# Lornatang/Real_ESRGAN-PyTorch

Measured on AMD Instinct MI355X. Metric: x4 SR train images/sec (256->1024), higher is better.
Workload: dtype f16; 1 GPU; RealESRNet x4 L1 train step, RRDBNet 23 blocks, LR 256^2 -> HR 1024^2, batch 16/GPU, degradation=hip, Adam+EMA, GradScaler; global_batch=16, parallelism=dp1

## Files before the change

### include/resr.h

```cpp
#ifndef RESR_H_
#define RESR_H_

#include <stddef.h>
#include <stdint.h>

#ifdef __cplusplus
extern "C" {
#endif

#define RESR_VERSION 3

typedef enum {
    RESR_OK = 0,
    RESR_ERR_ARG = -1,
    RESR_ERR_LAUNCH = -2,
    RESR_ERR_WORKSPACE = -3
} resr_status;

typedef enum { RESR_F16 = 0, RESR_F32 = 1, RESR_F16X2 = 2 } resr_dtype;

enum {
    RESR_CONV_LRELU = 1 << 0,
    RESR_CONV_UPSAMPLE_IN = 1 << 1,
    RESR_CONV_CLAMP01 = 1 << 2,
    RESR_CONV_OUT_NCHW_F32 = 1 << 3,
    RESR_CONV_MASK = 1 << 4,
    RESR_CONV_NO_BIAS = 1 << 5,
    RESR_CONV_AUX_BEFORE_MASK = 1 << 6,
    RESR_CONV_AUX_BEFORE_RES = 1 << 7,
    RESR_CONV_WRITE_SIGNBITS = 1 << 8,
    RESR_CONV_MASK_BITS = 1 << 9,
    RESR_CONV_OUT_SINGLE = 1 << 10,
    RESR_CONV_SINGLE_W16 = 1 << 11,
    RESR_CONV_MX_PAIRS = 1 << 12,
    RESR_CONV_MX_SIGNBITS = 1 << 13
};

typedef struct {
    int32_t n, h, w;
    int32_t cin;
    int32_t cin0;
    int32_t in0_stride;
    int32_t in1_stride;
    int32_t cout;
    int32_t cout_pad;
    int32_t out_stride;
    int32_t res0_stride, res1_stride, mask_stride;
    int32_t dtype;
    int32_t flags;
    float s0, t0, s1, t1, slope;
    int32_t in0_chunk_stride, in1_chunk_stride, out_chunk_stride;
    int32_t res0_chunk_stride, res1_chunk_stride, mask_chunk_stride;
    int64_t in0_lo_offset, in1_lo_offset, out_lo_offset, res0_lo_offset, res1_lo_offset;
    int32_t s2d_in_channels, s2d_out_channels, cout_groups;
    int32_t x2_pair_chunks;
    int32_t reserved2_;
    int64_t mask_lo_offset;
    int64_t in0_q_offset, in1_q_offset, out_q_offset, w_mx_offset;
} ResrConvDesc;

int resr_conv3x3(const ResrConvDesc* d, const void* in0, const void* in1, const void* w_packed,
                 const float* bias, const void* res0, const void* res1, const void* mask,
                 void* out, void* aux_out, void* stream);

size_t resr_conv3x3_chain_state_bytes(int32_t n, int32_t h, int32_t w);
int resr_conv3x3_chain(int32_t njobs, const ResrConvDesc* descs, const void* in0, const void* in1,
                       const void* const* packed_w, const float* const* bias, const void* const* mask,
                       void* const* out, void* const* aux_out, void* chain_state, size_t chain_state_bytes, void* stream);
// ... 210 lines not shown
```

### real_esrgan-pytorch_amd/_lib.py

```python
from __future__ import annotations

import ctypes as C
import os

_HERE = os.path.dirname(os.path.abspath(__file__))
LIB_PATH = os.environ.get("RESR_LIB_PATH") or os.path.join(_HERE, "csrc", "libresr_hip.so")

RESR_F16, RESR_F32, RESR_F16X2 = 0, 1, 2
CONV_LRELU, CONV_UPSAMPLE_IN, CONV_CLAMP01, CONV_OUT_NCHW_F32, CONV_MASK, CONV_NO_BIAS = 1, 2, 4, 8, 16, 32
CONV_AUX_BEFORE_MASK, CONV_AUX_BEFORE_RES = 64, 128
CONV_WRITE_SIGNBITS = 1 << 8
CONV_MASK_BITS = 1 << 9
CONV_OUT_SINGLE = 1 << 10
CONV_SINGLE_W16 = 1 << 11
X2_PLAN_GROWTH_F16_INFER, X2_PLAN_GROWTH_GRAD_F16, X2_PLAN_GROWTH_GRAD_STORE_F16, X2_PLAN_GROWTH_ACT_F16_WGRAD = 1, 2, 4, 8
X2_PLAN_GROWTH_ACT_G_HI_WGRAD = 16
X2_PLAN_GROWTH_W16_INFER = 32
X2_PLAN_MX_INFER = 64
X2_PLAN_MX_BWD = 128
X2_PLAN_F16_BACKWARD = 256
X2_PLAN_MX_WGRAD = 512
X2_PLAN_MX_TAIL = 1024
X2_PLAN_MX_TRAIN_FORWARD = 2048
X2_PLAN_OUTPUT_PARITY = (X2_PLAN_GROWTH_F16_INFER | X2_PLAN_GROWTH_W16_INFER | X2_PLAN_MX_INFER | X2_PLAN_F16_BACKWARD
# ... 6 lines not shown
    (512, 128 + 8, "MX_WGRAD (512) rides on MX_BWD (128: the gradient planes' q tensors) + GROWTH_ACT_F16_WGRAD (8: the stream chunks are the pair chunks)"),
    (1024, 512 + 128 + 8, "MX_TAIL (1024) extends MX_WGRAD (512) to the 4x-resolution tail"),
    (2048, 1 + 32 + 64 + 256, "MX_TRAIN_FORWARD (2048) runs the inference MX forward (1 + 32 + 64) in training, in front of the f16 backward pass (256)"),
)


def x2_plan_error(plan: int):
    if not 0 <= plan <= 4095:
        return ("x2_plan must be a bit set of X2_PLAN_GROWTH_F16_INFER (1) | X2_PLAN_GROWTH_GRAD_F16 (2) | X2_PLAN_GROWTH_GRAD_STORE_F16 (4) | "
                "X2_PLAN_GROWTH_ACT_F16_WGRAD (8) | X2_PLAN_GROWTH_ACT_G_HI_WGRAD (16) | X2_PLAN_GROWTH_W16_INFER (32) | X2_PLAN_MX_INFER (64) | "
                f"X2_PLAN_MX_BWD (128) | X2_PLAN_F16_BACKWARD (256) | X2_PLAN_MX_WGRAD (512) | X2_PLAN_MX_TAIL (1024) | X2_PLAN_MX_TRAIN_FORWARD (2048), got {plan}")
    if (plan & X2_PLAN_MX_BWD) and (plan & X2_PLAN_GROWTH_GRAD_STORE_F16):
        return f"x2_plan={plan}: MX_BWD (128) reads the growth-plane gradients as pairs; GROWTH_GRAD_STORE_F16 (4) stores them single"
    for bit, needs, text in X2_PLAN_RULES:
        if (plan & bit) and (plan & needs) != needs:
            return f"x2_plan={plan}: {text}"
    return None


def x2_plan_f16_backward(plan: int) -> bool:
    return bool(plan & X2_PLAN_F16_BACKWARD)


def x2_plan_packs_mx(plan: int, training: bool) -> bool:
    return bool(plan & ((X2_PLAN_MX_BWD | X2_PLAN_MX_TRAIN_FORWARD) if training else X2_PLAN_MX_INFER))


def x2_plan_layout_key(plan: int) -> int:
    return plan & (X2_PLAN_MX_INFER | X2_PLAN_MX_BWD | X2_PLAN_MX_WGRAD | X2_PLAN_MX_TAIL | X2_PLAN_MX_TRAIN_FORWARD)


CONV_MX_PAIRS = 1 << 12
CONV_MX_SIGNBITS = 1 << 13
RESR_VERSION = 3


class ConvDesc(C.Structure):
    _fields_ = [("n", C.c_int32), ("h", C.c_int32), ("w", C.c_int32),
                ("cin", C.c_int32), ("cin0", C.c_int32), ("in0_stride", C.c_int32), ("in1_stride", C.c_int32),
                ("cout", C.c_int32), ("cout_pad", C.c_int32), ("out_stride", C.c_int32),
                ("res0_stride", C.c_int32), ("res1_stride", C.c_int32), ("mask_stride", C.c_int32),
                ("dtype", C.c_int32), ("flags", C.c_int32),
                ("s0", C.c_float), ("t0", C.c_float), ("s1", C.c_float), ("t1", C.c_float), ("slope", C.c_float),
                ("in0_chunk_stride", C.c_int32), ("in1_chunk_stride", C.c_int32), ("out_chunk_stride", C.c_int32),
                ("res0_chunk_stride", C.c_int32), ("res1_chunk_stride", C.c_int32), ("mask_chunk_stride", C.c_int32),
                ("in0_lo_offset", C.c_int64), ("in1_lo_offset", C.c_int64), ("out_lo_offset", C.c_int64),
                ("res0_lo_offset", C.c_int64), ("res1_lo_offset", C.c_int64),
                ("s2d_in_channels", C.c_int32), ("s2d_out_channels", C.c_int32), ("cout_groups", C.c_int32),
                ("x2_pair_chunks", C.c_int32), ("reserved2_", C.c_int32), ("mask_lo_offset", C.c_int64),
                ("in0_q_offset", C.c_int64), ("in1_q_offset", C.c_int64), ("out_q_offset", C.c_int64), ("w_mx_offset", C.c_int64)]


class WgradDesc(C.Structure):
    _fields_ = [("n", C.c_int32), ("h", C.c_int32), ("w", C.c_int32),
                ("cin", C.c_int32), ("cin0", C.c_int32), ("in0_stride", C.c_int32), ("in1_stride", C.c_int32),
                ("cin_real", C.c_int32), ("cout", C.c_int32), ("cout_pad", C.c_int32), ("g_stride", C.c_int32),
                ("dtype", C.c_int32), ("flags", C.c_int32), ("splits", C.c_int32), ("scale", C.c_float),
                ("x_lo_offset", C.c_int64), ("g_lo_offset", C.c_int64), ("x_chunk_stride", C.c_int64), ("g_chunk_stride", C.c_int64)]


class PackChunk(C.Structure):
    _fields_ = [("src_off", C.c_int64), ("dst_off", C.c_int64), ("src_cout", C.c_int32), ("src_cin", C.c_int32),
                ("m_off", C.c_int32), ("m_count", C.c_int32), ("k_off", C.c_int32), ("k_count", C.c_int32),
                ("mt", C.c_int32), ("transposed", C.c_int32), ("scale", C.c_float), ("virtual4x4", C.c_int32),
                ("scale_ptr", C.c_void_p)]

# ... 173 lines not shown
```

### real_esrgan-pytorch_amd/csrc/conv3x3.h

```cpp
#pragma once
#include "common.h"

namespace resr {

struct ConvArgs {
    const char* in0;
    const char* in1;
    const char* w;
    const float* bias;
    const char* res0;
    const char* res1;
    const char* mask;
    char* out;
    uint8_t* aux;
    int n, h, w_, hs, ws;
    int cin, cin0;
    int in0_stride_b, in1_stride_b;
    int cout;
    int out_stride, res0_stride, res1_stride, mask_stride;
    size_t in0_chunk_b, in1_chunk_b;
    int out_chunk, res0_chunk, res1_chunk, mask_chunk;
    int flags;
    float s0, t0, s1, t1, slope;
    int tiles_x, tiles_y;
// ... 19 lines not shown
    const float* bias;
    char* out;
    void* aux;
    int cin;
    int dep;
    int kind;
    int w_mt, w_m;
    int pad_;
    const char* res0;
    const char* res1;
    float s0, t0, s1, t1;
    long out_lo, res0_lo, res1_lo;
    const char* w_mx;
    long out_q;
};
constexpr int kMaxChain = 6;
constexpr int kMaxBiasGroups = 8;
constexpr int kChainHdr = 16;
struct ChainArgs {
    int njobs;
    unsigned cap;
    unsigned* state;
    unsigned* host_errors;
    const char* nan16;
    int split[kMaxChain + 2];
    ChainJob job[kMaxChain];
};
struct ChainNone {};

inline double conv_algorithmic_bytes(const ConvArgs& a, size_t es) {
    const double px_out = (double)a.n * a.h * a.w_, px_in = (double)a.n * a.hs * a.ws;
    const int pair_ch = (es == 4 && a.pair_chunks > 0 && a.pair_chunks * 32 < a.cin) ? a.pair_chunks * 32 : a.cin;
    double b = px_in * (pair_ch * (double)es + (a.cin - pair_ch) * 2.0);
    const bool nchw = a.flags & RESR_CONV_OUT_NCHW_F32;
    b += px_out * a.cout * (nchw ? 4 : (es == 4 && a.out_single) ? 2 : es);
    if (a.flags & RESR_CONV_MASK) b += px_out * ((a.flags & RESR_CONV_MASK_BITS) ? ((a.cout + 31) / 32) * 4.0 : a.cout * (double)es);
    if (a.res0) b += px_out * a.cout * es;
    if (a.res1) b += px_out * a.cout * es;
    if (a.out_q) b += px_out * a.cout * 2.0;
    if (a.aux) b += px_out * ((a.flags & RESR_CONV_WRITE_SIGNBITS) ? ((a.cout + 31) / 32) * 4.0 : nchw ? a.cout : a.cout * (double)es);
    return b;
}

template <int SPP>
__device__ __forceinline__ int swz(int hx) {
    if constexpr (SPP == 4) return (hx >> 2) & 3;
    else return (hx >> 1) & 7;
}

template <typename T>
struct Frag;
template <>
struct Frag<half_t> {
    static __device__ __forceinline__ float16v mma(const uint4& a, const uint4& b, float16v c) {
        return __builtin_amdgcn_mfma_f32_32x32x16_f16(__builtin_bit_cast(half8, a),
                                                      __builtin_bit_cast(half8, b), c, 0, 0, 0);
    }
    static __device__ __forceinline__ float ld(const char* p, int idx) {
        return (float)reinterpret_cast<const half_t*>(p)[idx];
    }
};
template <>
struct Frag<float> {
    static __device__ __forceinline__ float16v mma(const uint4& a, const uint4& b, float16v c) {
        const float4v fa = __builtin_bit_cast(float4v, a), fb = __builtin_bit_cast(float4v, b);
        c = __builtin_amdgcn_mfma_f32_32x32x2f32(fa[0], fb[0], c, 0, 0, 0);
// ... 37 lines not shown
```

### real_esrgan-pytorch_amd/csrc/conv3x3.hip

```cpp
#include <stdlib.h>

#include <type_traits>

#include "conv3x3.h"

namespace resr {

template <typename T, int MT, int NT, int NW>
__global__ __launch_bounds__(64 * NW) void conv3x3_kernel(const ConvArgs a) {
    constexpr int NTHR = 64 * NW;
    constexpr int E = 16 / (int)sizeof(T);
    constexpr int SPP = 32 / E;
    constexpr int KS = SPP / 2;
    constexpr int PB = 32 * (int)sizeof(T);
    constexpr int TH = NW * NT, TW = 32, HH = TH + 2, HW = TW + 2;
    constexpr int NSLOT = HH * HW * SPP;
    constexpr int NS = (NSLOT + NTHR - 1) / NTHR;
    constexpr int BUF = HH * HW * PB;
    constexpr int WTAP = KS * MT * 1024;

    extern __shared__ __attribute__((aligned(16))) char smem[];

    const int tid = threadIdx.x, lane = tid & 63, wave = tid >> 6;
    const int bid = xcd_remap(blockIdx.x, gridDim.x);
// ... 234 lines not shown

int conv3x3_ws_f16(const ConvArgs& a, int mt, bool x2, hipStream_t stream);
bool conv3x3_ws_supported(const ConvArgs& a);
bool conv3x3_chain_device_ok();

int conv3x3_ws_chain_f16(const ConvArgs& a, const ChainJob* jobs, int njobs, const double* flop, const double* bytes, bool x2, void* state, size_t state_bytes,
                         hipStream_t stream);
static int conv3x3_route(const ResrConvDesc* d, ConvArgs& a, bool have_bias, bool have_in1, hipStream_t stream);

static int conv3x3_args(const ResrConvDesc* d, const void* in0, const void* in1, const void* w,
                        const float* bias, const void* res0, const void* res1, const void* mask,
                        void* out, void* aux, ConvArgs& a) {
    if (!d || !in0 || !w || !out) return fail(RESR_ERR_ARG, "conv3x3: null argument");
    if (d->cin <= 0 || (d->cin & 31) || (d->cin0 & 31) || d->cin0 <= 0 || d->cin0 > d->cin)
        return fail(RESR_ERR_ARG, "conv3x3: cin=%d cin0=%d must be positive multiples of 32", d->cin, d->cin0);
    if (d->cin0 < d->cin && !in1) return fail(RESR_ERR_ARG, "conv3x3: in1 missing for cin0 < cin");
    if (d->cout_pad != 32 && d->cout_pad != 64) return fail(RESR_ERR_ARG, "conv3x3: cout_pad=%d", d->cout_pad);
    if (d->cout <= 0 || d->cout > d->cout_pad) return fail(RESR_ERR_ARG, "conv3x3: cout=%d", d->cout);
    if (!(d->flags & RESR_CONV_OUT_NCHW_F32) && (d->cout & 3))
        return fail(RESR_ERR_ARG, "conv3x3: NHWC output needs cout %% 4 == 0");
    if (d->n <= 0 || d->h <= 0 || d->w <= 0) return fail(RESR_ERR_ARG, "conv3x3: empty shape");
    if ((d->flags & RESR_CONV_UPSAMPLE_IN) && ((d->h | d->w) & 1))
        return fail(RESR_ERR_ARG, "conv3x3: upsampled input needs even h,w");
    if ((d->flags & RESR_CONV_MASK) && !mask) return fail(RESR_ERR_ARG, "conv3x3: mask missing");
    if (d->flags & RESR_CONV_WRITE_SIGNBITS) {
        if (!aux || (d->cout & 7) || res0 || res1 ||
            (d->flags & (RESR_CONV_MASK | RESR_CONV_OUT_NCHW_F32 | RESR_CONV_CLAMP01 | RESR_CONV_AUX_BEFORE_MASK | RESR_CONV_AUX_BEFORE_RES)))
            return fail(RESR_ERR_ARG, "conv3x3: WRITE_SIGNBITS needs aux_out, cout %% 8 == 0 and a plain (bias/LeakyReLU) epilogue");
    }
    if (d->flags & RESR_CONV_MASK_BITS) {
        if (!(d->flags & RESR_CONV_MASK) || (d->cout & 7) || res0 || res1 || aux ||
            (d->flags & (RESR_CONV_OUT_NCHW_F32 | RESR_CONV_CLAMP01 | RESR_CONV_WRITE_SIGNBITS)))
            return fail(RESR_ERR_ARG, "conv3x3: MASK_BITS goes with MASK, cout %% 8 == 0, no residuals / aux");
    }
    const size_t es = elem_size(d->dtype);
    memset(&a, 0, sizeof(a));
    a.in0 = (const char*)in0; a.in1 = (const char*)in1; a.w = (const char*)w; a.bias = bias;
    a.res0 = (const char*)res0; a.res1 = (const char*)res1; a.mask = (const char*)mask;
    a.out = (char*)out; a.aux = (uint8_t*)aux;
    a.n = d->n; a.h = d->h; a.w_ = d->w;
    const bool up = d->flags & RESR_CONV_UPSAMPLE_IN;
    a.hs = up ? d->h / 2 : d->h; a.ws = up ? d->w / 2 : d->w;
    a.cin = d->cin; a.cin0 = d->cin0;
    a.in0_stride_b = (int)(d->in0_stride * es); a.in1_stride_b = (int)(d->in1_stride * es);
    a.cout = d->cout; a.out_stride = d->out_stride;
    a.res0_stride = d->res0_stride; a.res1_stride = d->res1_stride; a.mask_stride = d->mask_stride;
    auto chunk = [](int32_t v) { return v > 0 ? v : 32; };
    a.in0_chunk_b = (size_t)chunk(d->in0_chunk_stride) * es; a.in1_chunk_b = (size_t)chunk(d->in1_chunk_stride) * es;
    a.out_chunk = chunk(d->out_chunk_stride); a.res0_chunk = chunk(d->res0_chunk_stride);
    a.res1_chunk = chunk(d->res1_chunk_stride); a.mask_chunk = chunk(d->mask_chunk_stride);
    a.flags = d->flags & ~(RESR_CONV_OUT_SINGLE | RESR_CONV_SINGLE_W16 | RESR_CONV_MX_PAIRS | RESR_CONV_MX_SIGNBITS); a.s0 = d->s0; a.t0 = d->t0; a.s1 = d->s1; a.t1 = d->t1; a.slope = d->slope;
    a.s2d_c = 0; a.tap_c = 0; a.ngroups = 1; a.w_group_b = 0;
    a.pair_chunks = d->cin / 32; a.out_single = 0;
    a.mask_lo = (d->dtype == RESR_F16X2 && mask && (d->flags & RESR_CONV_MASK) && !(d->flags & RESR_CONV_MASK_BITS)) ? (long)d->mask_lo_offset : 0L;
    if (a.mask_lo < 0) return fail(RESR_ERR_ARG, "conv3x3: mask_lo_offset=%ld", a.mask_lo);
    if (d->dtype == RESR_F16X2) {
        if (d->x2_pair_chunks < 0 || d->x2_pair_chunks > d->cin / 32)
            return fail(RESR_ERR_ARG, "conv3x3: x2_pair_chunks=%d of %d chunks", d->x2_pair_chunks, d->cin / 32);
        if (d->x2_pair_chunks > 0) a.pair_chunks = d->x2_pair_chunks;
        if ((d->flags & RESR_CONV_SINGLE_W16) && a.pair_chunks * 32 < d->cin) a.single_stages = 1;
        if (d->flags & RESR_CONV_OUT_SINGLE) {
            if (d->flags & RESR_CONV_OUT_NCHW_F32) return fail(RESR_ERR_ARG, "conv3x3: OUT_SINGLE is an NHWC f16 output");
            a.out_single = 1;
        }
        if (d->in0_q_offset < 0 || d->in1_q_offset < 0 || d->out_q_offset < 0 || d->w_mx_offset < 0)
            return fail(RESR_ERR_ARG, "conv3x3: negative q / MX offset");
// ... 56 lines not shown
                     void* out, void* aux, hipStream_t stream) {
    ConvArgs a;
    const int rc = conv3x3_args(d, in0, in1, w, bias, res0, res1, mask, out, aux, a);
    if (rc) return rc;
    return conv3x3_route(d, a, bias != nullptr, in1 != nullptr, stream);
}

static int conv3x3_route(const ResrConvDesc* d, ConvArgs& a, bool have_bias, bool have_in1, hipStream_t stream) {
    const size_t es = elem_size(d->dtype);
    const void* in1 = have_in1 ? (const void*)a.in1 : nullptr;
    const void* res0 = a.res0;
    const void* res1 = a.res1;
    const int groups = d->cout_groups > 1 ? d->cout_groups : 1;
    (void)have_bias;
    const int mt = d->cout_pad / 32;
    if (d->dtype == RESR_F16X2) {
        const bool nchw = d->flags & RESR_CONV_OUT_NCHW_F32;
        const bool in1_pairs = in1 && d->cin0 < d->cin && a.pair_chunks * 32 > d->cin0;
        if (d->in0_lo_offset == 0 || (in1_pairs && d->in1_lo_offset == 0) || (!nchw && !a.out_single && d->out_lo_offset == 0) ||
            (res0 && d->res0_lo_offset == 0) || (res1 && d->res1_lo_offset == 0))
            return fail(RESR_ERR_ARG, "conv3x3: RESR_F16X2 needs the hi -> lo offset of every pair operand");
        a.in0_lo_b = (size_t)d->in0_lo_offset * es; a.in1_lo_b = (size_t)d->in1_lo_offset * es;
        a.out_lo = a.out_single ? 0L : (long)d->out_lo_offset; a.res0_lo = (long)d->res0_lo_offset; a.res1_lo = (long)d->res1_lo_offset;
        if (!conv3x3_ws_supported(a))
            return fail(RESR_ERR_ARG, "conv3x3: RESR_F16X2 needs tensors below 4 GB / 2^24 pixels and cout %% 8 == 0");
        if (a.mx && (a.s2d_c > 0 || a.tap_c > 0)) return fail(RESR_ERR_ARG, "conv3x3: RESR_CONV_MX_PAIRS with sparse taps");
        return conv3x3_ws_f16(a, mt, true, stream);
    }
    const long tiles4 = (long)((d->w + 31) / 32) * ((d->h + 15) / 16) * d->n;
    const bool big = tiles4 >= 512;
    if (d->dtype == RESR_F16) {
        static const char* old_env = getenv("RESR_CONV_ONE_ROLE");
        if (!old_env && conv3x3_ws_supported(a)) return conv3x3_ws_f16(a, mt, false, stream);
        if (groups > 1) return fail(RESR_ERR_ARG, "conv3x3: cout_groups > 1 needs the producer/consumer kernel's preconditions");
        if (mt == 1) return big ? launch_conv<half_t, 1, 2, 8>(a, stream) : launch_conv<half_t, 1, 2, 4>(a, stream);
        return launch_conv<half_t, 2, 2, 4>(a, stream);
    } else if (d->dtype == RESR_F32) {
        if (mt == 1) return launch_conv<float, 1, 2>(a, stream);
        return launch_conv<float, 2, 2>(a, stream);
    }
    return fail(RESR_ERR_ARG, "conv3x3: dtype=%d", d->dtype);
}

int conv3x3_block_dispatch(int njobs, const ResrConvDesc* d, const void* in0, const void* in1, const void* const* w,
                           const float* const* bias, const void* const* mask, void* const* out, void* const* aux,
                           const ResrConvDesc* d5, const void* w5, const float* bias5, const void* res0_5, const void* res1_5,
                           void* out5, void* chain_state, size_t chain_state_bytes, hipStream_t stream) {
    if (njobs <= 0 || njobs > 4 || !d) return fail(RESR_ERR_ARG, "conv3x3_chain: njobs=%d", njobs);
    ConvArgs a[4], a5;
    for (int j = 0; j < njobs; ++j) {
        const int rc = conv3x3_args(&d[j], in0, in1, w[j], bias ? bias[j] : nullptr, nullptr, nullptr, mask ? mask[j] : nullptr,
                                    out[j], aux ? aux[j] : nullptr, a[j]);
        if (rc) return rc;
    }
    if (d5) {
        const int rc = conv3x3_args(d5, in0, in1, w5, bias5, res0_5, res1_5, nullptr, out5, nullptr, a5);
        if (rc) return rc;
    }
    const char* no_chain = getenv("RESR_CONV_NO_CHAIN");
    const bool x2 = d[0].dtype == RESR_F16X2;
    bool ok = !no_chain && chain_state && njobs >= 2 && (d[0].dtype == RESR_F16 || x2) && conv3x3_chain_device_ok();
    if (ok && x2) {
        const size_t es2 = 2;
        for (int j = 0; j < njobs; ++j) {
            const bool in1_pairs = in1 && d[j].cin0 < d[j].cin && a[j].pair_chunks * 32 > d[j].cin0;
            if (d[j].dtype != RESR_F16X2 || d[j].in0_lo_offset == 0 || (d[j].out_lo_offset == 0 && !a[j].out_single) || (in1_pairs && d[j].in1_lo_offset == 0)) { ok = false; break; }
// ... 119 lines not shown
```

### real_esrgan-pytorch_amd/csrc/conv3x3_ws.h

```cpp
#pragma once
#include <stdlib.h>

#include <type_traits>

#include "conv3x3.h"

#ifndef RESR_TIMING_TAPS
#define RESR_TIMING_TAPS 9
#endif
#if defined(RESR_TRACE) && RESR_TRACE == 2
#define RESR_TRACE_STAMPS 192
#else
#define RESR_TRACE_STAMPS 64
#endif
#ifndef RESR_TIMING_VALU
#define RESR_TIMING_VALU 0
#endif

namespace resr {

static __device__ uint4 g_conv_zero16 = {0, 0, 0, 0};

extern unsigned long long* g_conv_trace;

// ... 165 lines not shown
            else a.trace[((blockIdx.x >> 4) * 2 + role) * RESR_TRACE_STAMPS + tk++] = __builtin_amdgcn_s_memrealtime();
        }
    };
    auto stamp_dump = [&](int role) {
        if constexpr (CH != 0) {
            if (a.trace && (blockIdx.x & 15) == 0 && blockIdx.x < 512 && lane == 0 && wave <= NWC)
                for (int i = 0; i < tk; ++i)
                    a.trace[((blockIdx.x >> 4) * 2 + role) * RESR_TRACE_STAMPS + i] = reinterpret_cast<const unsigned long long*>(smem + C::CHAIN_OFF + C::CHAIN_TRACE)[role * RESR_TRACE_STAMPS + i];
        }
    };

    if (wave == 0 || wave == NWC) stamp(wave == 0 ? 1 : 0);

    float* bias_lds = reinterpret_cast<float*>(smem + C::NHB * BUF);
    if (wave == 0) {
        const bool f_bias = !(a.flags & RESR_CONV_NO_BIAS) && a.bias != nullptr;
        bias_lds[lane] = (f_bias && lane < a.cout) ? a.bias[lane] * (X2 ? kLoScale : 1.f) : 0.f;
    }
    if constexpr (MT == 2 && CH == 0) {
        if (a.ngroups > 1 && !(a.flags & RESR_CONV_NO_BIAS) && a.bias != nullptr) {
            float* gb = reinterpret_cast<float*>(smem + C::GB_OFF);
            for (int i = tid; i < a.ngroups * 64 && i < kMaxBiasGroups * 64; i += C::NTHR)
                gb[i] = a.bias[i] * (X2 ? kLoScale : 1.f);
        }
    }
    if constexpr (CH) {
        float* cb = reinterpret_cast<float*>(smem + C::CHAIN_OFF);
        if (wave < kMaxChain && lane < 32) {
            const float* bp = wave < cj.njobs ? cj.job[wave].bias : nullptr;
            cb[wave * 32 + lane] = (bp && !(a.flags & RESR_CONV_NO_BIAS) && lane < a.cout) ? bp[lane] * (X2 ? kLoScale : 1.f) : 0.f;
        }
        if (wave == 0 && lane == 0) *reinterpret_cast<unsigned*>(smem + C::CHAIN_OFF + kMaxChain * 128) = 0u;
    }
    constexpr bool FAST = EPI == 0 || EPI == 2 || EPI == 6 || EPI == 16 || EPI == 33 || EPI == 128;
    if constexpr (EPI == 128) {
        if (wave == 1) reinterpret_cast<float*>(smem + C::LUT_OFF)[lane] = lane < a.cout ? a.prelu[lane] : 0.f;
    }
    if constexpr (FAST && EPI == 33) {
        if (wave == 1 && lane < 16) {
            float4v m;
#pragma unroll
            for (int r = 0; r < 4; ++r) m[r] = (((lane >> r) & 1) ? 1.f : a.slope) * (X2 ? kLoInv : 1.f);
            *reinterpret_cast<float4v*>(smem + C::LUT_OFF + lane * 16) = m;
        }
    }
    if (wave >= NWC) {
        const int pw = wave - NWC;
        if constexpr (C::NHB == 3) {
            const int ups3 = (a.flags & RESR_CONV_UPSAMPLE_IN) ? 1 : 0;
            constexpr int REM = NI - (NIP - 1) * NP;
            static_assert(NIP < 64, "vmcnt is 6 bits");
            unsigned cst[NIP], pix[NIP];
            unsigned long long val[NIP], inb[NIP];
            const unsigned lds_base = (unsigned)(size_t)(__attribute__((address_space(3))) char*)smem;
            auto dma_s = [&](const char* sbase, unsigned voff, unsigned dst, unsigned long long mask) {
                unsigned long long save;
                asm volatile("s_mov_b64 %0, exec\n\ts_mov_b64 exec, %1\n\ts_mov_b32 m0, %2\n\ts_nop 0\n\t"
                             "global_load_lds_dwordx4 %3, %4\n\ts_mov_b64 exec, %0"
                             : "=&s"(save) : "s"(mask), "s"(dst), "v"(voff), "s"(sbase) : "memory", "m0");
            };
            auto dma_v = [&](const char* src, unsigned dst, unsigned long long mask) {
                unsigned long long save;
                asm volatile("s_mov_b64 %0, exec\n\ts_mov_b64 exec, %1\n\ts_mov_b32 m0, %2\n\ts_nop 0\n\t"
                             "global_load_lds_dwordx4 %3, off\n\ts_mov_b64 exec, %0"
                             : "=&s"(save) : "s"(mask), "s"(dst), "v"(src) : "memory", "m0");
            };
#pragma unroll
// ... 692 lines not shown
            const int x = x0 + lx_e;
            const unsigned xc = (unsigned)(x < e.w_ ? x : e.w_ - 1);
            const bool f_lrelu = own && (e.flags & RESR_CONV_LRELU);
            const float2v sl2 = {e.slope, e.slope};
            const unsigned kh16 = (unsigned)kh_e * 16u;
            constexpr bool RESc = R0c || R1c;
            constexpr int NB = (RESc && MT == 2 && !(X2 && R1c)) ? 2 : 1;
            uint4v rr0[NB][MT][2], rr1[NB][MT][2];
            uint4v rr0l[X2 ? NB : 1][MT][2], rr1l[X2 ? NB : 1][MT][2];
            auto row_pix = [&](int t) {
                const int y = y0 + row0 + t;
                return ((unsigned)n * e.h + (unsigned)(y < e.h ? y : e.h - 1)) * e.w_ + xc;
            };
            auto piece_ok = [&](int m, int j) { return m * 32 + (2 * j + kh_e) * 8 < e.cout; };
            auto request = [&](int b, int t) {
                const unsigned p = row_pix(t);
#pragma unroll
                for (int m = 0; m < MT; ++m)
#pragma unroll
                    for (int j = 0; j < 2; ++j) {
                        const bool pair_ok = m * 32 + j * 16 < e.cout;
                        if (r0) {
                            const char* q0 = e.res0 + ((size_t)p * e.res0_stride + goff + (pair_ok ? (size_t)m * e.res0_chunk + j * 16 : (size_t)0)) * 2 + kh16;
                            rr0[b][m][j] = *reinterpret_cast<const uint4v*>(q0);
                            if constexpr (X2) rr0l[b][m][j] = *reinterpret_cast<const uint4v*>(q0 + e.res0_lo * 2);
                        }
                        if (r1) {
                            const char* q1 = e.res1 + ((size_t)p * e.res1_stride + goff + (pair_ok ? (size_t)m * e.res1_chunk + j * 16 : (size_t)0)) * 2 + kh16;
                            rr1[b][m][j] = *reinterpret_cast<const uint4v*>(q1);
                            if constexpr (X2) rr1l[b][m][j] = *reinterpret_cast<const uint4v*>(q1 + e.res1_lo * 2);
                        }
                    }
            };
            asm volatile("s_nop 7\n\ts_nop 7\n\ts_nop 3");
            if (r0 || r1) request(0, 0);
#pragma unroll
            for (int t = 0; t < NT; ++t) {
                const int y = y0 + row0 + t;
                const bool in_img = y < e.h && x < e.w_;
                const unsigned p = row_pix(t);
                const int b = NB == 2 ? (t & 1) : 0;
                if constexpr (NB == 2) {
                    if (t + 1 < NT) request((t + 1) & 1, t + 1);
                } else {
                    if ((r0 || r1) && t > 0) request(0, t);
                }
                char* const orow = e.out + ((size_t)p * e.out_stride + goff) * 2 + kh16;
#pragma unroll
                for (int m = 0; m < MT; ++m) {
                    unsigned sacc[2] = {0u, 0u};
                    unsigned wk = 0;
                    if constexpr (EMB) {
                        if (own) wk = mword[t][m] >> (kh_e * 8);
                    }
#pragma unroll
                    for (int j = 0; j < 2; ++j) {
                        float16v& A = acc[m][t];
                        float v0 = A[8 * j + 0], v1 = A[8 * j + 1], v2 = A[8 * j + 2], v3 = A[8 * j + 3];
                        float v4 = A[8 * j + 4], v5 = A[8 * j + 5], v6 = A[8 * j + 6], v7 = A[8 * j + 7];
                        permlane32_swap4(v0, v1, v2, v3, v4, v5, v6, v7);
                        float2v q[4] = {{v0, v1}, {v2, v3}, {v4, v5}, {v6, v7}};
                        if (EMB && own) {
                            const char* lut = smem + C::LUT_OFF;
                            const float4v ma = *reinterpret_cast<const float4v*>(lut + ((wk >> (16 * j)) & 15u) * 16);
                            const float4v mb = *reinterpret_cast<const float4v*>(lut + ((wk >> (16 * j + 4)) & 15u) * 16);
                            q[0] *= float2v{ma[0], ma[1]};
// ... 457 lines not shown
```

### real_esrgan-pytorch_amd/csrc/conv3x3_ws.hip

```cpp
#include <stdlib.h>

#include <mutex>

#include "conv3x3.h"

namespace resr {

unsigned long long* g_conv_trace = nullptr;
void conv_trace_set(void* p) { g_conv_trace = (unsigned long long*)p; }

int conv3x3_ws_mt1(const ConvArgs& a, int tile_rows, hipStream_t stream);
int conv3x3_ws_mt2(const ConvArgs& a, int tile_rows, hipStream_t stream);
int conv3x3_ws_x2_mt1(const ConvArgs& a, int tile_rows, hipStream_t stream);
int conv3x3_ws_x2_mt2(const ConvArgs& a, int tile_rows, hipStream_t stream);
int conv3x3_ws_mx_mt1(const ConvArgs& a, int tile_rows, hipStream_t stream);
int conv3x3_ws_mx_mt2(const ConvArgs& a, int tile_rows, hipStream_t stream);

bool conv3x3_chain_device_ok() {
    static int ok_dev[kMaxDevices] = {0};
    int dev = 0;
    if (hipGetDevice(&dev) != hipSuccess || dev < 0 || dev >= kMaxDevices) return false;
    if (!ok_dev[dev]) {
        hipDeviceProp_t prop;
        ok_dev[dev] = (hipGetDeviceProperties(&prop, dev) == hipSuccess && prop.multiProcessorCount == 256) ? 1 : -1;
// ... 92 lines not shown
            if (hipEventCreateWithFlags(&c.ev, hipEventDisableTiming) != hipSuccess ||
                hipHostMalloc(&hp, 64, hipHostMallocMapped) != hipSuccess || hipHostGetDevicePointer(&dp, hp, 0) != hipSuccess ||
                hipGetSymbolAddress(&np, HIP_SYMBOL(g_conv_nan16)) != hipSuccess || !np)
                return fail(RESR_ERR_LAUNCH, "conv3x3_chain: per-device set-up failed");
            memset(hp, 0, 64);
            c.err_host = (unsigned*)hp; c.err_dev = (unsigned*)dp; c.nan16 = (const char*)np;
            c.init = true;
        }
        hipStreamCaptureStatus cap = hipStreamCaptureStatusNone;
        if (hipStreamIsCapturing(stream, &cap) != hipSuccess) cap = hipStreamCaptureStatusNone;
        const bool capturing = cap == hipStreamCaptureStatusActive;
        if (!capturing) {
            if (c.owned && c.owner != stream && hipStreamWaitEvent(stream, c.ev, 0) != hipSuccess)
                return fail(RESR_ERR_LAUNCH, "conv3x3_chain: hipStreamWaitEvent");
            c.owner = stream;
            c.owned = true;
        }
        cj.state = (unsigned*)state;
        cj.cap = (unsigned)(state_bytes / sizeof(unsigned) - kChainHdr);
        cj.host_errors = c.err_dev;
        cj.nan16 = c.nan16;
        cj.njobs = njobs;
        memcpy(cj.split, split, sizeof(split));
        double f = 0, b = 0;
        for (int j = 0; j < njobs; ++j) { cj.job[j] = jobs[j]; f += flop[j]; b += bytes[j]; }
        for (int j = njobs; j < kMaxChain; ++j) cj.job[j] = jobs[njobs - 1];
        const int kind = (a.flags & RESR_CONV_MASK_BITS) ? 2 : (a.flags & RESR_CONV_WRITE_SIGNBITS) ? 1 : 0;
        const int rc = conv3x3_ws_chain_launch(a, cj, rows, kind, x2, f, b, stream);
        if (rc == RESR_OK && !capturing && hipEventRecord(c.ev, stream) != hipSuccess) return fail(RESR_ERR_LAUNCH, "conv3x3_chain: hipEventRecord");
        return rc;
    }
}

int conv3x3_ws_f16(const ConvArgs& a, int mt, bool x2, hipStream_t stream) {
    static const int rows1[] = {16, 8}, rows2[] = {16, 8};
    if (mt == 2 && (a.s2d_c > 0 || a.tap_c > 0) && !a.res0 && !a.res1 && !a.mask && !a.aux &&
        !(a.flags & ~(RESR_CONV_LRELU | RESR_CONV_NO_BIAS)) && a.cin0 == a.cin && (!(a.flags & RESR_CONV_LRELU) || (a.slope >= 0.f && a.slope <= 1.f)))
        return conv3x3_ws_sparse(a, 8, a.s2d_c > 0 ? 1 : 2, x2, stream);
    if (x2 && a.mx) {
        if (mt == 1) return conv3x3_ws_mx_mt1(a, pick_rows(a, rows1, 2), stream);
        return conv3x3_ws_mx_mt2(a, pick_rows(a, rows2, 2), stream);
    }
    if (x2) {
        if (mt == 1) return conv3x3_ws_x2_mt1(a, pick_rows(a, rows1, 2), stream);
        return conv3x3_ws_x2_mt2(a, pick_rows(a, rows2, 2), stream);
    }
    if (mt == 1) return conv3x3_ws_mt1(a, pick_rows(a, rows1, 2), stream);
    return conv3x3_ws_mt2(a, pick_rows(a, rows2, 2), stream);
}

}
```

### real_esrgan-pytorch_amd/csrc/generator.hip

```cpp
#include <stdlib.h>
#include <vector>

#include "common.h"
#include "wgrad.h"

namespace resr {

int conv3x3_dispatch(const ResrConvDesc*, const void*, const void*, const void*, const float*, const void*,
                     const void*, const void*, void*, void*, hipStream_t);
size_t wgrad_batch_partial_bytes(const WgradConv*, int, int, int);
int conv3x3_block_dispatch(int njobs, const ResrConvDesc* d, const void* in0, const void* in1, const void* const* w,
                           const float* const* bias, const void* const* mask, void* const* out, void* const* aux,
                           const ResrConvDesc* d5, const void* w5, const float* bias5, const void* res0_5, const void* res1_5,
                           void* out5, void* chain_state, size_t chain_state_bytes, hipStream_t stream);
size_t conv3x3_chain_state_bytes(int, int, int);
int wgrad_batch(const WgradConv*, int, int, int, int, int, int, int, float*, hipStream_t);
int wgrad_batch_jobs(const WgradConv*, int, int);
int wgrad_batch_quads(const WgradConv*, int, int);
int wgrad_tile_rows(int dtype);
int wgrad_x2_products();
int absmax_dispatch(const float*, long, unsigned*, int, hipStream_t);
int nchw_to_nhwc_q_dispatch(const float*, void*, int, int, int, int, int, int, int, const uint8_t*, hipStream_t, long, const unsigned*, long);
int nhwc_to_nchw_scaled_dispatch(const void*, float*, int, int, int, int, int, int, int, hipStream_t, long, const unsigned*);
int sumpool2x2_dispatch(const void*, void*, const void*, int, int, int, int, int, float, hipStream_t, long, long);
// ... 547 lines not shown
}

int generator_backward(const ResrGeneratorDesc* d, const float* gy, const float* params, const void* packed,
                       void* workspace, size_t workspace_bytes, float* grad, float* gx, hipStream_t st,
                       void* const* events, int n_events) {
    (void)params;
    Plan p;
    if (!build_plan(d, p)) return RESR_ERR_ARG;
    if (n_events != 0 && (!events || n_events != d->n_blocks + 2))
        return fail(RESR_ERR_ARG, "generator_backward: grad_ready_events needs n_blocks + 2 = %d events, got %d", d->n_blocks + 2, n_events);
    auto ready = [&](int i) -> int {
        if (n_events == 0) return RESR_OK;
        if (!events[i]) return fail(RESR_ERR_ARG, "generator_backward: null event %d", i);
        if (hipEventRecord((hipEvent_t)events[i], st) != hipSuccess) return fail(RESR_ERR_LAUNCH, "generator_backward: hipEventRecord");
        return RESR_OK;
    };
    if (!d->training) return fail(RESR_ERR_ARG, "generator_backward: forward was not run with training=1");
    if (!gy || !packed || !workspace || !grad) return fail(RESR_ERR_ARG, "generator_backward: null argument");
    Bufs b;
    carve(p, (char*)workspace, b);
    if (b.total > workspace_bytes) return fail(RESR_ERR_WORKSPACE, "generator_backward: workspace %zu < %zu", workspace_bytes, b.total);
    const X2Plan& xp = p.x2;
    const int dt = xp.f16_backward ? (int)RESR_F16 : d->dtype;
    Plan pb = p;
    pb.d.dtype = dt;
    const size_t es = elem_size(dt);
    const bool x2 = dt == RESR_F16X2;
    const size_t wes = es * (x2 ? 3 : 1);
    const int wm = x2 ? wgrad_x2_products() : 1;
    const char* no_prescale = getenv("RESR_X2_NO_GRAD_PRESCALE");
    const char* pre_t = getenv("RESR_X2_GRAD_PRESCALE_LOG2");
    const int pre_log2 = pre_t ? atoi(pre_t) : 6;
    const unsigned* gsc = (dt != RESR_F32 && !no_prescale) ? b.gscale : nullptr;
    const char* pk = (const char*)packed;
    const int N = d->n, h = p.h, w = p.w;
    const int H4 = 4 * h, W4 = 4 * w, H2 = 2 * h, W2 = 2 * w;
    if ((long)N * h * w * 32 * 16 > 0x7fffffffL) return fail(RESR_ERR_ARG, "generator: batch x resolution too large for 32-bit chunk strides");
    const int plane = N * h * w * 32;
    const int pl2 = 4 * plane, pl4 = 16 * plane;
    auto LO = [&](long planes, long pl) -> long { return x2 ? planes * pl : 0; };
    const long lo_ws = LO(6, plane), lo_t = LO(2, plane), lo_gs = LO(4, plane), lo_2 = LO(2, pl2), lo_4 = LO(2, pl4), lo_g4 = LO(1, pl4);
    const long lo_xin = x2 ? (long)N * h * w * p.ci_pad : 0;

    auto wconv = [&](const ConvSpec& c, const void* x0, int cin, int s0, const void* g, int gstride, float scale,
                     long x_lo, long g_lo) {
        WgradConv wc;
        wc.x0 = x0; wc.cin = cin; wc.in0_stride = s0; wc.cin_real = c.cin;
        wc.g = g; wc.cout = c.cout; wc.cout_pad = c.cout_pad; wc.g_stride = gstride;
        wc.x_chunk_stride = wc.g_chunk_stride = 0;
        wc.x_lo_off = x_lo; wc.g_lo_off = g_lo; wc.x_s2d_c = 0; wc.g_lo_bias_only = 0;
        wc.dw = grad + c.w_off; wc.db = grad + c.b_off; wc.scale = scale;
        wc.unscale = gsc;
        return wc;
    };
    auto wgrad_run = [&](const WgradConv* wc, int nconv, int hh, int ww, int flags) -> int {
        const int njobs = wgrad_batch_jobs(wc, nconv, dt);
        const int splits = splits_for(pb, njobs, hh, ww, x2 ? wgrad_batch_quads(wc, nconv, dt) : 0);
        if (wgrad_batch_partial_bytes(wc, nconv, splits, dt) > b.partial_bytes)
            return fail(RESR_ERR_WORKSPACE, "wgrad slab buffer too small");
        return wgrad_batch(wc, nconv, N, hh, ww, dt, flags, splits, b.partial, st);
    };
    auto wgrad = [&](const ConvSpec& c, int hh, int ww, const void* x0, int cin, int s0, const void* g, int gstride,
                     int flags, float scale, long x_chunk, long g_chunk, long x_lo, long g_lo, long x_q = 0, long g_q = 0) -> int {
        WgradConv wc = wconv(c, x0, cin, s0, g, gstride, scale, x_lo, g_lo);
        wc.x_chunk_stride = x_chunk; wc.g_chunk_stride = g_chunk;
        wc.x_q_off = x_q; wc.g_q_off = g_q;
// ... 5 lines not shown
        cd.in0_lo_offset = lo0; cd.in1_lo_offset = lo1; cd.out_lo_offset = lo_out;
        return cd;
    };

    if (gsc) RUN(absmax_dispatch(gy, (long)N * d->out_channels * H4 * W4, b.gscale, pre_log2, st));
    RUN(nchw_to_nhwc_q_dispatch(gy, b.g4, N, d->out_channels, H4, W4, 1, 32, dt, b.ymask, st, lo_g4, gsc, xp.mx_tail ? 2 * lo_g4 : 0L));
    const char* pk_mx = xp.mx_bwd ? pk + generator_mx_offset(d) : nullptr;
    auto MXT = [&](ResrConvDesc& cd, size_t pk_off, long in_q, long out_q) {
        if (!xp.mx_tail) return;
        cd.flags |= RESR_CONV_MX_PAIRS;
        cd.in0_q_offset = in_q; cd.out_q_offset = out_q;
        cd.w_mx_offset = (int64_t)((pk_mx + pk_off * 2) - (pk + pk_off * wes));
    };
    {
        const ConvSpec& c = p.convs[p.i_conv4];
        RUN(wgrad(c, H4, W4, b.c3, 64, 32, b.g4, 32, 0, 1.f, pl4, 0, lo_4, lo_g4, xp.mx_tail ? 2 * lo_4 : 0, xp.mx_tail ? 2 * lo_g4 : 0));
        ResrConvDesc cd = dgrad(H4, W4, 32, 32, 32, 0, 64, 64, 32, RESR_CONV_MASK | RESR_CONV_MASK_BITS, lo_g4, 0, lo_4);
        cd.out_chunk_stride = pl4;
        MXT(cd, p.pk_bwd_conv4, 2 * lo_g4, 2 * lo_4);
        RUN(conv3x3_dispatch(&cd, b.g4, nullptr, pk + p.pk_bwd_conv4 * wes, nullptr, nullptr, nullptr, b.bits_c3, b.gA, nullptr, st));
    }
    {
        const ConvSpec& c = p.convs[p.i_conv3];
        RUN(wgrad(c, H4, W4, b.u2, 64, 32, b.gA, 32, 0, 1.f, pl4, pl4, lo_4, lo_4, xp.mx_tail ? 2 * lo_4 : 0, xp.mx_tail ? 2 * lo_4 : 0));
        ResrConvDesc cd = dgrad(H4, W4, 64, 32, 64, 0, 64, 64, 32, RESR_CONV_MASK | RESR_CONV_MASK_BITS, lo_4, 0, lo_4);
        cd.in0_chunk_stride = pl4; cd.out_chunk_stride = pl4;
        MXT(cd, p.pk_bwd_conv3, 2 * lo_4, 2 * lo_4);
        RUN(conv3x3_dispatch(&cd, b.gA, nullptr, pk + p.pk_bwd_conv3 * wes, nullptr, nullptr, nullptr, b.bits_u2, b.gB, nullptr, st));
    }
    if (debug_stop() == 1) return RESR_OK;
    {
        const ConvSpec& c = p.convs[p.i_up2];
        RUN(wgrad(c, H4, W4, b.u1, 64, 32, b.gB, 32, RESR_CONV_UPSAMPLE_IN, 1.f, pl2, pl4, lo_2, lo_4, xp.mx_tail ? 2 * lo_2 : 0, xp.mx_tail ? 2 * lo_4 : 0));
        ResrConvDesc cd = dgrad(H4, W4, 64, 32, 64, 0, 64, 64, 32, 0, lo_4, 0, lo_4);
        cd.in0_chunk_stride = pl4; cd.out_chunk_stride = pl4;
        MXT(cd, p.pk_bwd_up2, 2 * lo_4, 0);
        RUN(conv3x3_dispatch(&cd, b.gB, nullptr, pk + p.pk_bwd_up2 * wes, nullptr, nullptr, nullptr, nullptr, b.gA, nullptr, st));
        for (int q = 0; q < 2; ++q)
            RUN(sumpool2x2_dispatch(b.gA + (size_t)q * pl4 * es, b.gM1 + (size_t)q * pl2 * es, b.u1 + (size_t)q * pl2 * es,
                                    N, H2, W2, 32, dt, 0.2f, st, lo_4, lo_2));
    }
    if (debug_stop() == 2) return RESR_OK;
    {
        const ConvSpec& c = p.convs[p.i_up1];
        RUN(wgrad(c, H2, W2, b.feat, 64, 32, b.gM1, 32, RESR_CONV_UPSAMPLE_IN, 1.f, plane, pl2, lo_t, lo_2));
        ResrConvDesc cd = dgrad(H2, W2, 64, 32, 64, 0, 64, 64, 32, 0, lo_2, 0, lo_2);
        cd.in0_chunk_stride = pl2; cd.out_chunk_stride = pl2;
        RUN(conv3x3_dispatch(&cd, b.gM1, nullptr, pk + p.pk_bwd_up1 * wes, nullptr, nullptr, nullptr, nullptr, b.gA, nullptr, st));
        for (int q = 0; q < 2; ++q)
            RUN(sumpool2x2_dispatch(b.gA + (size_t)q * pl2 * es, b.gF + (size_t)q * plane * es, nullptr, N, h, w, 32, dt, 0.2f, st,
                                    lo_2, lo_t));
    }
    if (debug_stop() == 3) return RESR_OK;
    int cur = 0;
    {
        const ConvSpec& c = p.convs[p.i_conv2];
        RUN(wgrad(c, h, w, b.trunk_out, 64, 32, b.gF, 32, 0, 1.f, plane, plane, lo_t, lo_t));
        ResrConvDesc cd = dgrad(h, w, 64, 32, 64, 0, 64, 64, 32, 0, lo_t, 0, lo_t);
        cd.in0_chunk_stride = plane; cd.out_chunk_stride = plane;
        if (xp.mx_bwd) cd.out_q_offset = 2 * lo_t;
        RUN(conv3x3_dispatch(&cd, b.gF, nullptr, pk + p.pk_bwd_conv2 * wes, nullptr, nullptr, nullptr, nullptr, b.gT[0], nullptr, st));
    }
    auto MXB = [&](ResrConvDesc& cd, size_t pk_off, long out_q) {
        if (!xp.mx_bwd) return;
        cd.flags |= RESR_CONV_MX_PAIRS;
        cd.x2_pair_chunks = 0;
        cd.in0_q_offset = 2 * lo_t; cd.in1_q_offset = 2 * lo_gs; cd.out_q_offset = out_q;
        cd.w_mx_offset = (int64_t)((pk_mx + pk_off * 2) - (pk + pk_off * wes));
    };
    RUN(ready(0));
    int e_idx = 0;
    const bool batch_rrdb = 78 * wm <= kWgradMaxJobs && !getenv("RESR_WGRAD_PER_BLOCK");
    WgradConv wc[15];
    for (int r = p.nrdb - 1; r >= 0; --r) {
        const int pos = r % 3;
        if (pos == 2) e_idx = cur;
        const char* gin = b.gT[cur];
        const char* act = b.ws[r];
        char* gS = b.gS[pos];
        const float fold = pos == 2 ? 0.04f : 0.2f;
        WgradConv* wcb = wc + (batch_rrdb ? 5 * pos : 0);
// ... 65 lines not shown
```

Before: 131.4 images/sec.

## Fuse 2x2 sum-pool and LeakyReLU mask into upsample dgrad epilogue

Adds a POOL2X2_OUT epilogue to the warp-specialized f16 conv kernel. It sums each 2x2 output cell in registers using DPP lane swaps, optionally applies the pooled LeakyReLU mask, and writes the quarter-resolution gradient directly. The two upsample-conv backward passes now use it when the dtype is f16, which removes the full-resolution gradient write and the separate sumpool kernels' read-back. The cost is extra epilogue register pressure and a narrower set of supported configurations.

Result: no change. 132.1 images/sec, median of 6 (+0.6%).

```diff
diff --git a/include/resr.h b/include/resr.h
--- a/include/resr.h
+++ b/include/resr.h
@@ -33,7 +33,8 @@
     RESR_CONV_OUT_SINGLE = 1 << 10,
     RESR_CONV_SINGLE_W16 = 1 << 11,
     RESR_CONV_MX_PAIRS = 1 << 12,
-    RESR_CONV_MX_SIGNBITS = 1 << 13
+    RESR_CONV_MX_SIGNBITS = 1 << 13,
+    RESR_CONV_POOL2X2_OUT = 1 << 14
 };
 
 typedef struct {
diff --git a/real_esrgan-pytorch_amd/_lib.py b/real_esrgan-pytorch_amd/_lib.py
--- a/real_esrgan-pytorch_amd/_lib.py
+++ b/real_esrgan-pytorch_amd/_lib.py
@@ -62,6 +62,7 @@
 
 CONV_MX_PAIRS = 1 << 12
 CONV_MX_SIGNBITS = 1 << 13
+CONV_POOL2X2_OUT = 1 << 14
 RESR_VERSION = 3
 
 
diff --git a/real_esrgan-pytorch_amd/csrc/conv3x3.h b/real_esrgan-pytorch_amd/csrc/conv3x3.h
--- a/real_esrgan-pytorch_amd/csrc/conv3x3.h
+++ b/real_esrgan-pytorch_amd/csrc/conv3x3.h
@@ -75,6 +75,8 @@
     const double px_out = (double)a.n * a.h * a.w_, px_in = (double)a.n * a.hs * a.ws;
     const int pair_ch = (es == 4 && a.pair_chunks > 0 && a.pair_chunks * 32 < a.cin) ? a.pair_chunks * 32 : a.cin;
     double b = px_in * (pair_ch * (double)es + (a.cin - pair_ch) * 2.0);
+    if (a.flags & RESR_CONV_POOL2X2_OUT)
+        return b + px_out / 4 * a.cout * (double)es * ((a.flags & RESR_CONV_MASK) ? 2 : 1);
     const bool nchw = a.flags & RESR_CONV_OUT_NCHW_F32;
     b += px_out * a.cout * (nchw ? 4 : (es == 4 && a.out_single) ? 2 : es);
     if (a.flags & RESR_CONV_MASK) b += px_out * ((a.flags & RESR_CONV_MASK_BITS) ? ((a.cout + 31) / 32) * 4.0 : a.cout * (double)es);
diff --git a/real_esrgan-pytorch_amd/csrc/conv3x3.hip b/real_esrgan-pytorch_amd/csrc/conv3x3.hip
--- a/real_esrgan-pytorch_amd/csrc/conv3x3.hip
+++ b/real_esrgan-pytorch_amd/csrc/conv3x3.hip
@@ -290,6 +290,12 @@
         if (!(d->flags & RESR_CONV_MASK) || (d->cout & 7) || res0 || res1 || aux ||
             (d->flags & (RESR_CONV_OUT_NCHW_F32 | RESR_CONV_CLAMP01 | RESR_CONV_WRITE_SIGNBITS)))
             return fail(RESR_ERR_ARG, "conv3x3: MASK_BITS goes with MASK, cout %% 8 == 0, no residuals / aux");
+    }
+    if (d->flags & RESR_CONV_POOL2X2_OUT) {
+        if (d->dtype != RESR_F16 || d->cout != 64 || d->cout_pad != 64 || ((d->h | d->w) & 1) || res0 || res1 || aux || d->out_q_offset != 0 ||
+            d->cout_groups > 1 || d->s2d_in_channels > 0 || d->s2d_out_channels > 0 ||
+            (d->flags & ~(RESR_CONV_POOL2X2_OUT | RESR_CONV_NO_BIAS | RESR_CONV_MASK)))
+            return fail(RESR_ERR_ARG, "conv3x3: POOL2X2_OUT needs f16, cout = cout_pad = 64, even h and w, a plain epilogue (bias, pooled f16 mask) and no out_q / groups / sparse taps");
     }
     const size_t es = elem_size(d->dtype);
     memset(&a, 0, sizeof(a));
@@ -412,6 +418,7 @@
     if (d->dtype == RESR_F16) {
         static const char* old_env = getenv("RESR_CONV_ONE_ROLE");
         if (!old_env && conv3x3_ws_supported(a)) return conv3x3_ws_f16(a, mt, false, stream);
+        if (d->flags & RESR_CONV_POOL2X2_OUT) return fail(RESR_ERR_ARG, "conv3x3: POOL2X2_OUT needs the producer/consumer kernel's preconditions");
         if (groups > 1) return fail(RESR_ERR_ARG, "conv3x3: cout_groups > 1 needs the producer/consumer kernel's preconditions");
         if (mt == 1) return big ? launch_conv<half_t, 1, 2, 8>(a, stream) : launch_conv<half_t, 1, 2, 4>(a, stream);
         return launch_conv<half_t, 2, 2, 4>(a, stream);
diff --git a/real_esrgan-pytorch_amd/csrc/conv3x3_ws.h b/real_esrgan-pytorch_amd/csrc/conv3x3_ws.h
--- a/real_esrgan-pytorch_amd/csrc/conv3x3_ws.h
+++ b/real_esrgan-pytorch_amd/csrc/conv3x3_ws.h
@@ -221,7 +221,8 @@
         }
         if (wave == 0 && lane == 0) *reinterpret_cast<unsigned*>(smem + C::CHAIN_OFF + kMaxChain * 128) = 0u;
     }
-    constexpr bool FAST = EPI == 0 || EPI == 2 || EPI == 6 || EPI == 16 || EPI == 33 || EPI == 128;
+    constexpr bool FAST = EPI == 0 || EPI == 2 || EPI == 6 || EPI == 16 || EPI == 33 || EPI == 128 || EPI == 256 || EPI == 257;
+    static_assert(!(EPI & 256) || (EPI <= 257 && sizeof(T) == 2 && MT == 2 && (NT & 1) == 0 && !X2 && !SP && !CH), "pooled epilogue: f16, cout 64, even rows per wave");
     if constexpr (EPI == 128) {
         if (wave == 1) reinterpret_cast<float*>(smem + C::LUT_OFF)[lane] = lane < a.cout ? a.prelu[lane] : 0.f;
     }
@@ -980,6 +981,88 @@
                         }
                     }
             };
+            if constexpr ((EPI & 256) != 0) {
+                constexpr bool PM = (EPI & 1) != 0;
+                constexpr int NC = NT / 2;
+                const int ho = e.h >> 1, wo = e.w_ >> 1;
+                const unsigned xo = xc >> 1;
+                auto cell_pix = [&](int c) {
+                    const int yo = (y0 + row0 + 2 * c) >> 1;
+                    return ((unsigned)n * ho + (unsigned)(yo < ho ? yo : ho - 1)) * wo + xo;
+                };
+                uint4v mk[PM ? NC : 1][MT][2];
+                if constexpr (PM) {
+                    const char* const mbase = ep->mask;
+                    const int m_stride = ep->mask_stride, m_chunk = ep->mask_chunk;
+#pragma unroll
+                    for (int c = 0; c < NC; ++c) {
+                        const unsigned p2 = cell_pix(c);
+#pragma unroll
+                        for (int m = 0; m < MT; ++m)
+#pragma unroll
+                            for (int j = 0; j < 2; ++j)
+                                mk[c][m][j] = *reinterpret_cast<const uint4v*>(mbase + ((size_t)p2 * m_stride + (size_t)m * m_chunk + j * 16) * 2 + kh16);
+                    }
+                }
+                asm volatile("s_nop 7\n\ts_nop 7\n\ts_nop 3");
+                float2v ps[NC][MT][2][4];
+#pragma unroll
+                for (int m = 0; m < MT; ++m)
+#pragma unroll
+                    for (int j = 0; j < 2; ++j) {
+                        unsigned dd[NT][4], pd[NT][4];
+#pragma unroll
+                        for (int t = 0; t < NT; ++t) {
+                            float16v& A = acc[m][t];
+                            float v0 = A[8 * j + 0], v1 = A[8 * j + 1], v2 = A[8 * j + 2], v3 = A[8 * j + 3];
+                            float v4 = A[8 * j + 4], v5 = A[8 * j + 5], v6 = A[8 * j + 6], v7 = A[8 * j + 7];
+                            permlane32_swap4(v0, v1, v2, v3, v4, v5, v6, v7);
+                            const float2v q[4] = {{v0, v1}, {v2, v3}, {v4, v5}, {v6, v7}};
+#pragma unroll
+                            for (int k = 0; k < 4; ++k) {
+                                dd[t][k] = __builtin_bit_cast(unsigned, __builtin_convertvector(q[k], half2v));
+                                pd[t][k] = (unsigned)__builtin_amdgcn_update_dpp(0, (int)dd[t][k], 0xB1, 0xf, 0xf, true);
+                            }
+                        }
+#pragma unroll
+                        for (int c = 0; c < NC; ++c)
+#pragma unroll
+                            for (int k = 0; k < 4; ++k) {
+                                const unsigned q4[4] = {dd[2 * c][k], pd[2 * c][k], dd[2 * c + 1][k], pd[2 * c + 1][k]};
+                                float2v s = {0.f, 0.f};
+#pragma unroll
+                                for (int i = 0; i < 4; ++i) s = float2v{mixfma_lo(q4[i], 1.f, s[0]), mixfma_hi(q4[i], 1.f, s[1])};
+                                ps[c][m][j][k] = s;
+                            }
+                    }
+#pragma unroll
+                for (int c = 0; c < NC; ++c) {
+                    const bool cell_ok = (lx_e & 1) == 0 && x < e.w_ && y0 + row0 + 2 * c < e.h;
+                    char* const orow = e.out + (size_t)cell_pix(c) * e.out_stride * 2 + kh16;
+#pragma unroll
+                    for (int m = 0; m < MT; ++m)
+#pragma unroll
+                        for (int j = 0; j < 2; ++j) {
+                            uint4v d;
+#pragma unroll
+                            for (int k = 0; k < 4; ++k) {
+                                float2v s = ps[c][m][j][k];
+                                if constexpr (PM) {
+                                    const unsigned mu = mk[c][m][j][k];
+                                    const half2v mh = __builtin_bit_cast(half2v, mu);
+                                    const float2v sq = s * sl2;
+                                    s = float2v{mh[0] > (_Float16)0 ? s[0] : sq[0], mh[1] > (_Float16)0 ? s[1] : sq[1]};
+                                }
+                                d[k] = __builtin_bit_cast(unsigned, __builtin_convertvector(s, half2v));
+                            }
+                            if (cell_ok) *reinterpret_cast<uint4v*>(orow + ((size_t)m * e.out_chunk + j * 16) * 2) = d;
+                        }
+                }
+                group_bias(tile + tile_step);
+                init_acc();
+                if (wave == 0) stamp(1);
+                continue;
+            }
             asm volatile("s_nop 7\n\ts_nop 7\n\ts_nop 3");
             if (r0 || r1) request(0, 0);
 #pragma unroll
diff --git a/real_esrgan-pytorch_amd/csrc/conv3x3_ws.hip b/real_esrgan-pytorch_amd/csrc/conv3x3_ws.hip
--- a/real_esrgan-pytorch_amd/csrc/conv3x3_ws.hip
+++ b/real_esrgan-pytorch_amd/csrc/conv3x3_ws.hip
@@ -148,8 +148,11 @@
     }
 }
 
+int conv3x3_ws_pool(const ConvArgs& a, hipStream_t stream);
+
 int conv3x3_ws_f16(const ConvArgs& a, int mt, bool x2, hipStream_t stream) {
     static const int rows1[] = {16, 8}, rows2[] = {16, 8};
+    if (a.flags & RESR_CONV_POOL2X2_OUT) return (mt == 2 && !x2) ? conv3x3_ws_pool(a, stream) : fail(RESR_ERR_ARG, "conv3x3: POOL2X2_OUT is an f16 cout-64 pass");
     if (mt == 2 && (a.s2d_c > 0 || a.tap_c > 0) && !a.res0 && !a.res1 && !a.mask && !a.aux &&
         !(a.flags & ~(RESR_CONV_LRELU | RESR_CONV_NO_BIAS)) && a.cin0 == a.cin && (!(a.flags & RESR_CONV_LRELU) || (a.slope >= 0.f && a.slope <= 1.f)))
         return conv3x3_ws_sparse(a, 8, a.s2d_c > 0 ? 1 : 2, x2, stream);
diff --git a/real_esrgan-pytorch_amd/csrc/conv3x3_ws_pool.hip b/real_esrgan-pytorch_amd/csrc/conv3x3_ws_pool.hip
--- /dev/null
+++ b/real_esrgan-pytorch_amd/csrc/conv3x3_ws_pool.hip
@@ -0,0 +1,10 @@
+#include "conv3x3_ws.h"
+
+namespace resr {
+
+int conv3x3_ws_pool(const ConvArgs& a, hipStream_t stream) {
+    if (a.flags & RESR_CONV_MASK) return launch_ws_epi<half_t, 2, 4, 4, 257>(a, stream);
+    return launch_ws_epi<half_t, 2, 4, 4, 256>(a, stream);
+}
+
+}
diff --git a/real_esrgan-pytorch_amd/csrc/generator.hip b/real_esrgan-pytorch_amd/csrc/generator.hip
--- a/real_esrgan-pytorch_amd/csrc/generator.hip
+++ b/real_esrgan-pytorch_amd/csrc/generator.hip
@@ -603,6 +603,7 @@
     const char* pre_t = getenv("RESR_X2_GRAD_PRESCALE_LOG2");
     const int pre_log2 = pre_t ? atoi(pre_t) : 6;
     const unsigned* gsc = (dt != RESR_F32 && !no_prescale) ? b.gscale : nullptr;
+    const bool tail_fused = dt == RESR_F16 && !getenv("RESR_TAIL_UNFUSED");
     const char* pk = (const char*)packed;
     const int N = d->n, h = p.h, w = p.w;
     const int H4 = 4 * h, W4 = 4 * w, H2 = 2 * h, W2 = 2 * w;
@@ -674,10 +675,12 @@
     {
         const ConvSpec& c = p.convs[p.i_up2];
         RUN(wgrad(c, H4, W4, b.u1, 64, 32, b.gB, 32, RESR_CONV_UPSAMPLE_IN, 1.f, pl2, pl4, lo_2, lo_4, xp.mx_tail ? 2 * lo_2 : 0, xp.mx_tail ? 2 * lo_4 : 0));
-        ResrConvDesc cd = dgrad(H4, W4, 64, 32, 64, 0, 64, 64, 32, 0, lo_4, 0, lo_4);
-        cd.in0_chunk_stride = pl4; cd.out_chunk_stride = pl4;
+        ResrConvDesc cd = dgrad(H4, W4, 64, 32, 64, 0, 64, 64, 32, tail_fused ? RESR_CONV_POOL2X2_OUT | RESR_CONV_MASK : 0, lo_4, 0, lo_4);
+        cd.in0_chunk_stride = pl4; cd.out_chunk_stride = tail_fused ? pl2 : pl4;
+        if (tail_fused) { cd.mask_stride = 32; cd.mask_chunk_stride = pl2; }
         MXT(cd, p.pk_bwd_up2, 2 * lo_4, 0);
-        RUN(conv3x3_dispatch(&cd, b.gB, nullptr, pk + p.pk_bwd_up2 * wes, nullptr, nullptr, nullptr, nullptr, b.gA, nullptr, st));
+        RUN(conv3x3_dispatch(&cd, b.gB, nullptr, pk + p.pk_bwd_up2 * wes, nullptr, nullptr, nullptr, tail_fused ? b.u1 : nullptr, tail_fused ? b.gM1 : b.gA, nullptr, st));
+        if (!tail_fused)
         for (int q = 0; q < 2; ++q)
             RUN(sumpool2x2_dispatch(b.gA + (size_t)q * pl4 * es, b.gM1 + (size_t)q * pl2 * es, b.u1 + (size_t)q * pl2 * es,
                                     N, H2, W2, 32, dt, 0.2f, st, lo_4, lo_2));
@@ -686,9 +689,10 @@
     {
         const ConvSpec& c = p.convs[p.i_up1];
         RUN(wgrad(c, H2, W2, b.feat, 64, 32, b.gM1, 32, RESR_CONV_UPSAMPLE_IN, 1.f, plane, pl2, lo_t, lo_2));
-        ResrConvDesc cd = dgrad(H2, W2, 64, 32, 64, 0, 64, 64, 32, 0, lo_2, 0, lo_2);
-        cd.in0_chunk_stride = pl2; cd.out_chunk_stride = pl2;
-        RUN(conv3x3_dispatch(&cd, b.gM1, nullptr, pk + p.pk_bwd_up1 * wes, nullptr, nullptr, nullptr, nullptr, b.gA, nullptr, st));
+        ResrConvDesc cd = dgrad(H2, W2, 64, 32, 64, 0, 64, 64, 32, tail_fused ? RESR_CONV_POOL2X2_OUT : 0, lo_2, 0, lo_2);
+        cd.in0_chunk_stride = pl2; cd.out_chunk_stride = tail_fused ? plane : pl2;
+        RUN(conv3x3_dispatch(&cd, b.gM1, nullptr, pk + p.pk_bwd_up1 * wes, nullptr, nullptr, nullptr, nullptr, tail_fused ? b.gF : b.gA, nullptr, st));
+        if (!tail_fused)
         for (int q = 0; q < 2; ++q)
             RUN(sumpool2x2_dispatch(b.gA + (size_t)q * pl2 * es, b.gF + (size_t)q * plane * es, nullptr, N, h, w, 32, dt, 0.2f, st,
                                     lo_2, lo_t));
```
